# jimmc414/semantic_merge

Hardware: AMD Instinct MI355X
Metric: op-log compose+conflict throughput (ops/s), 100M-op logs, 1/2/4/8 GPUs (higher is better)
Workload: dtype u64; 1 GPU; c3: one merge of 100,000,000 ops (100,000,000 per GPU), 1,000,000 symbols, 64 ops/ms, seed 11; n_ops_per_gpu=100000000, n_ops_total=100000000, n_sym=1000000, composed_ops=99989720, conflicts=5140, plan=presorted, parallelism=single GPU

## Files before the change

semantic_merge_amd/csrc/smx_compose.hip:

```cpp
#include <algorithm>
#include <atomic>
#include <chrono>
#include <cstring>
#include <mutex>
#include <string>
#include <vector>

#include "smx_sort.h"
#include "smx_window.h"
#include "smx_small.h"
#include "smx_batch.h"
#include "smx_tables.h"


static thread_local std::string g_err;
static int set_err(int code, const std::string& msg) {
  g_err = msg;
  return code;
}
int smx_set_error(int code, const char* msg) { return set_err(code, msg ? msg : ""); }
#define HIP_TRY(x)                                                                 \
  do {                                                                             \
    hipError_t _e = (x);                                                           \
    if (_e != hipSuccess)                                                          \
// ... 1052 lines not shown
  const u64 nskip = M->n_skip;
  const u64 nmv = min(M->kcnt[KMOVE], E.n);
  const u64 nP = E.n - nmv;
  const u64 nR = min(M->kcnt[KREN], nP);
  const u64 nout = E.n - nskip, nRk = nR - nskip;
  auto gsrc = [&](i32 j) -> i32 {
    if (E.src_map) return E.src_map[j];
    return (u64)j < E.na_loc ? (i32)(E.src_a + j) : (i32)(E.src_b + ((i64)j - (i64)E.na_loc));
  };
  const FinPack FP = fin_pack_of(M->vbits, E.allow_pack != 0);
  const int lane = threadIdx.x & (WAVE - 1);
  const u64 w0 = (((u64)blockIdx.x * BLOCK + threadIdx.x) / WAVE) * EMIT_WT;
  if (w0 + EMIT_WT <= nmv || w0 >= nout || nP == 0) return;
  u64 kk = 0;
  {
    const u64 o0 = w0 > nmv ? w0 - nmv : 0;
    if (o0 < nRk) {
      u64 lo = 0, hi = nskip;
      while (lo < hi) {
        const u64 mid = (lo + hi) >> 1;
        if ((u64)E.skiplist[mid] - mid < o0) lo = mid + 1;
        else hi = mid;
      }
      kk = lo;
    }
  }
  u64 pp[EMIT4_STEPS][4];
  bool vec[EMIT4_STEPS];
#pragma unroll
  for (int j = 0; j < EMIT4_STEPS; ++j) {
    const u64 b = w0 + (u64)j * 4 * WAVE;
    const u64 o = b + 4 * (u64)lane;
    u64 add[4] = {0, 0, 0, 0};
    const u64 k0 = kk;
    if (b + 4 * WAVE > nmv && (b > nmv ? b - nmv : 0) < nRk) {
      const u64 ohi = b + 4 * WAVE - 1 - nmv;
      while (kk < nskip) {
        const u64 sj = (u64)(u32)__builtin_amdgcn_readfirstlane((int)E.skiplist[kk]) - kk;
        if (sj > ohi) break;
#pragma unroll
        for (int u = 0; u < 4; ++u) add[u] += (o + u >= nmv ? o + u - nmv : 0) >= sj;
        ++kk;
      }
    }
#pragma unroll
    for (int u = 0; u < 4; ++u) {
      const u64 ou = o + u;
      const u64 op = ou >= nmv ? ou - nmv : 0;
      const bool ok = ou >= nmv && ou < nout;
      pp[j][u] = !ok ? 0 : (op < nRk ? op + k0 + add[u] : op + nskip);
    }
    vec[j] = o >= nmv && o + 3 < nout && pp[j][3] == pp[j][0] + 3;
  }
  i32 src[EMIT4_STEPS][4];
  u32 sy[EMIT4_STEPS][4];
#pragma unroll
  for (int j = 0; j < EMIT4_STEPS; ++j) {
    if (vec[j]) {
      const ev4u s4 = __builtin_nontemporal_load(reinterpret_cast<const ev4u_a4*>(&E.tsrc[pp[j][0]]));
      const ev4u y4 = __builtin_nontemporal_load(reinterpret_cast<const ev4u_a4*>(&E.tsym[pp[j][0]]));
      src[j][0] = (i32)s4.x, src[j][1] = (i32)s4.y, src[j][2] = (i32)s4.z, src[j][3] = (i32)s4.w;
      sy[j][0] = y4.x, sy[j][1] = y4.y, sy[j][2] = y4.z, sy[j][3] = y4.w;
    } else {
#pragma unroll
      for (int u = 0; u < 4; ++u) {
        src[j][u] = NTLD(&E.tsrc[pp[j][u]]);
        sy[j][u] = NTLD(&E.tsym[pp[j][u]]);
      }
    }
#pragma unroll
    for (int u = 0; u < 4; ++u) sy[j][u] = min(sy[j][u], E.smax);
  }
#pragma unroll
  for (int j = 0; j < EMIT4_STEPS; ++j) {
    int4 F[4];
    if (FP.packed) {
      u64 x[4];
#pragma unroll
      for (int u = 0; u < 4; ++u) x[u] = fin_word(FP, E.fin, sy[j][u]);
#pragma unroll
      for (int u = 0; u < 4; ++u) F[u] = fin_decode(FP, x[u]);
    } else {
#pragma unroll
      for (int u = 0; u < 4; ++u) F[u] = E.fin[sy[j][u]];
    }
    const u64 o = w0 + (u64)j * 4 * WAVE + 4 * (u64)lane;
    i32 vo[4], va[4], vf[4], vc[4];
#pragma unroll
    for (int u = 0; u < 4; ++u) {
      const bool ren = o + u >= nmv && o + u - nmv < nRk;
      vo[u] = gsrc(src[j][u]);
      va[u] = F[u].x;
      vf[u] = F[u].y;
      vc[u] = ren ? -1 : F[u].z;
    }
    if (o >= nmv && o + 3 < nout) {
      NTST((ev4i{vo[0], vo[1], vo[2], vo[3]}), reinterpret_cast<ev4i*>(&E.out_order[o]));
      NTST((ev4i{va[0], va[1], va[2], va[3]}), reinterpret_cast<ev4i*>(&E.out_addr[o]));
      NTST((ev4i{vf[0], vf[1], vf[2], vf[3]}), reinterpret_cast<ev4i*>(&E.out_file[o]));
      NTST((ev4i{vc[0], vc[1], vc[2], vc[3]}), reinterpret_cast<ev4i*>(&E.out_ctx[o]));
    } else {
#pragma unroll
      for (int u = 0; u < 4; ++u) {
        if (o + u >= nmv && o + u < nout) {
          E.out_order[o + u] = vo[u];
          E.out_addr[o + u] = va[u];
          E.out_file[o + u] = vf[u];
          E.out_ctx[o + u] = vc[u];
        }
      }
    }
  }
}

__global__ void k_mv_init(const u32* __restrict__ msym, u64 nMv, u64* __restrict__ keys, u32* __restrict__ vals) {
  for (u64 j = (u64)blockIdx.x * BLOCK + threadIdx.x; j < nMv; j += (u64)gridDim.x * BLOCK) {
    keys[j] = msym[j] & SYM_MASK;
    vals[j] = (u32)j;
  }
}

__global__ void k_mv_fix(const u64* __restrict__ keys, const u32* __restrict__ vals, u64 nMv,
                         const u32* __restrict__ msym, const u64* __restrict__ mvpre, u64 n_sym,
                         i32* __restrict__ out_addr, i32* __restrict__ out_file) {
  for (u64 j = (u64)blockIdx.x * BLOCK + threadIdx.x; j < nMv; j += (u64)gridDim.x * BLOCK) {
    if (j != 0 && keys[j - 1] == keys[j]) continue;
    i32 ra = -1, rf = -1;
    if (mvpre && keys[j] < n_sym) {
      const u64 pa = mvpre[keys[j]], pf = mvpre[n_sym + keys[j]];
      if (pa) ra = (i32)(u32)pa - 1;
      if (pf) rf = (i32)(u32)pf - 1;
    }
    for (u64 i = j; i < nMv && keys[i] == keys[j]; ++i) {
      const u32 T = vals[i];
      const u32 f = msym[T];
      if (f & MS_HAS_A) ra = out_addr[T];
      else out_addr[T] = ra;
      if (f & MS_HAS_F) rf = out_file[T];
      else out_file[T] = rf;
    }
  }
}


struct Layout {
  size_t off[64];
  size_t total;
};

enum Buf {
  B_META, B_BND, B_WCNT, B_WOFF, B_STS, B_SHI, B_SLO, B_PERM, B_RKEY, B_RVAL, B_RK2, B_RV2,
  B_RHIST, B_PART, B_MSYM, B_TSRC, B_TSYM, B_RSTR, B_WREN, B_WBND, B_CSLOT, B_WCAND, B_WCANDB,
  B_WCOFF, B_CAND, B_Q, B_PM, B_NCONF, B_NREAL, B_COFF, B_SKIPBITS, B_SKIPLIST,
  B_TABA, B_TABF, B_TABR, B_FIN, B_REC, B_TBHIST, B_CCNT, B_TSUM, B_SMP, B_N
};

static i64 max_windows(i64 nn) { return SMX_CEIL_DIV(nn, (i64)WIN_TGT_MIN) + 2; }

static Layout layout(i64 na, i64 nb, i64 n_sym) {
  const i64 n = na + nb;
  const i64 nn = n > 0 ? n : 1;
  const i64 W = max_windows(nn);
  size_t sz[B_N];
  sz[B_META] = sizeof(ComposeMeta);
  sz[B_BND] = (size_t)(W + 1) * 2 * 8;
  sz[B_WCNT] = (size_t)NCNT * W * 4;
  sz[B_WOFF] = (size_t)NCNT * W * 4;
  sz[B_STS] = sz[B_SHI] = sz[B_SLO] = (size_t)nn * 8;
  sz[B_PERM] = (size_t)nn * 4;
  sz[B_RKEY] = (size_t)nn * 8;
  sz[B_RVAL] = (size_t)nn * 4;
  sz[B_RK2] = (size_t)nn * 8;
  sz[B_RV2] = (size_t)nn * 4;
  sz[B_RHIST] = radix_hist_bytes(nn);
  sz[B_PART] = (size_t)SCAN_NB * 8;
  sz[B_MSYM] = sz[B_TSRC] = sz[B_TSYM] = sz[B_RSTR] = (size_t)nn * 4;
  sz[B_WREN] = (size_t)W * 2 * 4;
  sz[B_WBND] = sz[B_WCAND] = sz[B_WCANDB] = sz[B_WCOFF] = (size_t)W * 4;
  sz[B_CSLOT] = sz[B_CAND] = sz[B_Q] = sz[B_PM] = sz[B_NCONF] = sz[B_NREAL] = sz[B_COFF] = (size_t)nn * 4;
  sz[B_SKIPBITS] = (size_t)(SMX_CEIL_DIV(nn, (i64)64) + 1) * 8;
  sz[B_SKIPLIST] = (size_t)nn * 4;
  const i64 ns = n_sym > 0 ? n_sym : 1;
  sz[B_TABA] = sz[B_TABF] = sz[B_TABR] = (size_t)ns * 4;
  sz[B_FIN] = (size_t)ns * 16;
  sz[B_REC] = (size_t)nn * 4;
  sz[B_TBHIST] = (size_t)(TB_MAXBK + 1) * SMX_CEIL_DIV(nn, (i64)TB_TILE) * 4;
  sz[B_CCNT] = (size_t)2 * SMX_N_KINDS * (SMX_CEIL_DIV(nn, (i64)256) + 2) * 4;
  sz[B_SMP] = (size_t)(SMX_CEIL_DIV(nn, (i64)CH) + 4) * 8;
  sz[B_TSUM] = (size_t)2 * SMX_N_KINDS * (SMX_CEIL_DIV(nn, (i64)CH * CS_TILE) + 2) * 4;
  Layout L{};
  size_t acc = 0;
  for (int i = 0; i < B_N; ++i) {
    L.off[i] = acc;
    acc += (sz[i] + 255) & ~(size_t)255;
  }
  L.total = acc;
  return L;
}


static int grid_for(i64 n, int per_block_items = BLOCK) {
  i64 g = SMX_CEIL_DIV(n > 0 ? n : 1, (i64)per_block_items);
  if (g > 4096) g = 4096;
  return (int)g;
}

extern "C" int smx_compose_workspace_bytes(int64_t n_a, int64_t n_b, int64_t n_sym, size_t* bytes) {
  if (!bytes || n_a < 0 || n_b < 0 || n_sym < 0) return set_err(SMX_E_ARG, "bad argument");
  *bytes = layout(n_a, n_b, n_sym).total;
  return SMX_OK;
}

struct Ctx {
  const smx_ops* ops;
  const smx_compose_out* out;
  hipStream_t st;
  Layout L{};
  char* base;
  i64 na, nb, n, n_sym;
  i64 src_a, src_b;
  StageTimer* tm;
  const i32* src_map = nullptr;
  u64* hrec = nullptr;
  u64 hseq = 0;
  template <typename T>
  T* ws(int b) const { return (T*)(base + L.off[b]); }
};

#if SMX_DIAG
static void* g_phase_dbg = nullptr;
static size_t g_phase_dbg_bytes = 0;
extern "C" int smx_debug_phase_buffer(void* p, size_t bytes) {
  g_phase_dbg = p;
  g_phase_dbg_bytes = bytes;
  return SMX_OK;
}
#else
static constexpr void* g_phase_dbg = nullptr;
static constexpr size_t g_phase_dbg_bytes = 0;
#endif

static WinArgs win_args(const Ctx& C) {
  WinArgs P{};
  P.kind = C.ops->kind;
  P.sym = C.ops->sym;
  P.v0 = C.ops->v0;
  P.v1 = C.ops->v1;
  P.na = C.na;
  P.nb = C.nb;
  P.bgap = C.ops->b_gap;
  P.n_sym = C.n_sym;
  P.src_a = C.src_a;
  P.src_b = C.src_b;
  P.src_map = C.src_map;
  P.bnd = C.ws<i64>(B_BND);
  P.woff = C.ws<u32>(B_WOFF);
  P.meta = C.ws<ComposeMeta>(B_META);
  P.out_order = C.out->order;
  P.out_addr = C.out->addr;
  P.out_file = C.out->file;
  P.out_ctx = C.out->ctx;
  P.msym = C.ws<u32>(B_MSYM);
  P.tsrc = C.ws<i32>(B_TSRC);
  P.tsym = C.ws<u32>(B_TSYM);
  P.Rstr = C.ws<i32>(B_RSTR);
  P.wren = C.ws<u32>(B_WREN);
  P.wbnd = C.ws<u32>(B_WBND);
  P.cslot = C.ws<u32>(B_CSLOT);
  P.wcand = C.ws<u32>(B_WCAND);
  return P;
}

static WalkArgs walk_args(const Ctx& C, const smx_shard* sh) {
  WalkArgs Wk{};
  Wk.tsrc = C.ws<i32>(B_TSRC);
  Wk.tsym = C.ws<u32>(B_TSYM);
  Wk.v0 = C.ops->v0;
  Wk.wren = C.ws<u32>(B_WREN);
  Wk.wbnd = C.ws<u32>(B_WBND);
  Wk.meta = C.ws<ComposeMeta>(B_META);
  Wk.na_cap = (u64)C.na;
  Wk.nb_cap = (u64)C.nb;
  Wk.bgap = C.ops->b_gap;
  Wk.src_a = C.src_a;
  Wk.src_b = C.src_b;
  Wk.src_map = C.src_map;
  Wk.halo_dev = sh ? sh->halo_dev : nullptr;
  for (int b = 0; b < 2; ++b) {
    Wk.halo_sym[b] = sh ? sh->halo_sym[b] : nullptr;
    Wk.halo_cls[b] = sh ? sh->halo_cls[b] : nullptr;
    Wk.halo_src[b] = sh ? sh->halo_src[b] : nullptr;
    Wk.halo_n[b] = sh && sh->halo_sym[b] ? (u64)sh->halo_n[b] : 0;
    Wk.halo_more[b] = sh ? sh->halo_more[b] : 0;
  }
  Wk.stage = C.ws<u32>(B_RK2);
  Wk.sok = C.ws<u32>(B_RV2);
  Wk.stage_cap = RS_CONF ? (u64)(C.n > 0 ? C.n : 1) * 2 / (RS_CONF ? RS_W : 1) : 0;
  return Wk;
}

#ifndef SMX_WALK_LB
#define SMX_WALK_LB 0
#endif
static int launch_walk(const Ctx& C, const smx_shard* sh) {
  hipStream_t st = C.st;
  ComposeMeta* meta = C.ws<ComposeMeta>(B_META);
  const i64 n = C.n;
  u64* skipbits = C.ws<u64>(B_SKIPBITS);
  u32* skiplist = C.ws<u32>(B_SKIPLIST);
  u32* part = C.ws<u32>(B_PART);
  const u64 nskipw = (u64)SMX_CEIL_DIV(n, (i64)64) + 1;
  const WalkArgs Wk = walk_args(C, sh);
  u32* cslot = C.ws<u32>(B_CSLOT);
  u32* wcand = C.ws<u32>(B_WCAND);
  u32* wtot = C.ws<u32>(B_WCANDB);
  u32* wcoff = C.ws<u32>(B_WCOFF);
  u32* cand = C.ws<u32>(B_CAND);
  u32* q = C.ws<u32>(B_Q);
  u32* pm = C.ws<u32>(B_PM);
  u32* nconf = C.ws<u32>(B_NCONF);
  u32* nreal = C.ws<u32>(B_NREAL);
  u32* coff = C.ws<u32>(B_COFF);
  u32* nconf32 = (u32*)&meta->n_conf_loc;
  u32* ncand32 = (u32*)&meta->n_cand;
  const u64* ncand_dev = &meta->n_cand;
  const i64 Wmax = max_windows(n);
#ifndef WALK_GSMALL
#define WALK_GSMALL 256
#endif
  const int gsmall = WALK_GSMALL;
  const bool lb_cc = SMX_WALK_LB && !sh && Wmax <= WALK_CC_FUSED_MAXW;
  const bool lb_cl = SMX_WALK_LB && !sh && n <= WALK_FUSED_MAXN;
  if (lb_cc)
    hipLaunchKernelGGL(k_boundary_cc, dim3(grid_for(Wmax)), dim3(BLOCK), 0, st, Wk, meta, cslot, wcand, wtot,
                       skipbits, nskipw, wcoff, (u64)Wmax, ncand32, cand);
  else
    hipLaunchKernelGGL(k_boundary, dim3(grid_for(Wmax)), dim3(BLOCK), 0, st, Wk, meta, cslot, wcand, wtot, skipbits,
// ... 45 lines not shown
  A.ncap = (u64)C.n;
  A.width = 1u;
  A.nbk = 1u;
  A.smax = (u32)(C.n_sym - 1);
  return A;
}

static bool tb_geometry(const Ctx& C, u64* width_o, u64* nbk_o) {
  u64 width = SMX_CEIL_DIV((u64)C.n_sym, (u64)TB_NBK_TGT);
  if (width < 1) width = 1;
  if (width > TB_WIDTH) width = TB_WIDTH;
  *width_o = width;
  *nbk_o = SMX_CEIL_DIV((u64)C.n_sym, width);
  return *nbk_o <= TB_MAXBK;
}

static int launch_tb_prescatter(const Ctx& C) {
  u64 width, nbk;
  if (!tb_geometry(C, &width, &nbk)) return SMX_OK;
  TbArgs A = tb_args(C);
  A.width = (u32)width;
  A.nbk = (u32)nbk;
  A.keep_skip = 1u;
  hipLaunchKernelGGL(k_tb_scatter, dim3((int)SMX_CEIL_DIV((u64)C.n, (u64)TB_TILE)), dim3(TB_NT), 0, C.st, A,
                     C.ws<u32>(B_TBHIST), C.ws<u32>(B_REC));
  HIP_TRY(hipGetLastError());
  return SMX_OK;
}

static int launch_tables(const Ctx& C, void* part_tab, u32 tag, int tagbits, bool* bucketed,
                         bool prescattered = false) {
  hipStream_t st = C.st;
  const i64 n = C.n;
  int4* fin = C.ws<int4>(B_FIN);
  *bucketed = false;
  const i64 n_sym = C.n_sym;
  TbArgs A = tb_args(C);
  u64 width, nbk;
  if (tb_geometry(C, &width, &nbk)) {
    *bucketed = true;
    A.width = (u32)width;
    A.nbk = (u32)nbk;
    const int nblk = (int)SMX_CEIL_DIV((u64)n, (u64)TB_TILE);
    u32* lst = C.ws<u32>(B_TBHIST);
    u32* rec = C.ws<u32>(B_REC);
    if (prescattered) {
      A.keep_skip = 1u;
      hipLaunchKernelGGL(k_tb_unskip, dim3(1024), dim3(BLOCK), 0, st, A, lst, rec, C.ws<u32>(B_SKIPLIST));
    } else {
      hipLaunchKernelGGL(k_tb_scatter, dim3(nblk), dim3(TB_NT), 0, st, A, lst, rec);
    }
    hipLaunchKernelGGL(k_tb_reduce, dim3(nbk), dim3(TBR_NT), 0, st, A, lst, rec, n_sym, fin,
                       PartTab{part_tab, tag, tagbits, C.ws<ComposeMeta>(B_META)});
  } else {
    u32* tabA = C.ws<u32>(B_TABA);
    u32* tabF = C.ws<u32>(B_TABF);
    u32* tabR = C.ws<u32>(B_TABR);
    int rc;
    if ((rc = zero_async(tabA, (size_t)n_sym * 4, st)) || (rc = zero_async(tabF, (size_t)n_sym * 4, st)) ||
        (rc = zero_async(tabR, (size_t)n_sym * 4, st)))
      return rc;
    hipLaunchKernelGGL(k_tab_atomic, dim3(grid_for(n)), dim3(BLOCK), 0, st, A, tabA, tabF, tabR);
    hipLaunchKernelGGL(k_finalize, dim3(grid_for(n_sym)), dim3(BLOCK), 0, st, A, tabA, tabF, tabR, n_sym, fin,
                       PartTab{part_tab, tag, tagbits, C.ws<ComposeMeta>(B_META)});
  }
  HIP_TRY(hipGetLastError());
  return SMX_OK;
}

static int launch_emit(const Ctx& C, bool packable, const smx_shard* sh) {
  hipStream_t st = C.st;
  ComposeMeta* meta = C.ws<ComposeMeta>(B_META);
  const i64 n = C.n;
  EmitArgs E{C.ws<i32>(B_TSRC), C.ws<u32>(B_TSYM), C.ws<u64>(B_SKIPBITS), C.ws<u32>(B_SKIPLIST),
             C.ws<int4>(B_FIN), meta, (u64)n, (u32)(C.n_sym - 1), packable ? 1 : 0, (u64)C.na, C.src_a,
             C.src_b, C.src_map, C.out->order, C.out->addr, C.out->file, C.out->ctx, C.out->counts, sh ? 0 : 1,
             sh ? nullptr : C.hrec, C.hseq};
  const i64 ewaves = SMX_CEIL_DIV(n, (i64)EMIT_WT);
  const bool al16 = ((uintptr_t)C.out->order | (uintptr_t)C.out->addr | (uintptr_t)C.out->file |
                     (uintptr_t)C.out->ctx) % 16 == 0;
  if (EMIT_VEC && al16)
    hipLaunchKernelGGL(k_emit4, dim3(SMX_CEIL_DIV(ewaves, (i64)NWAVES)), dim3(BLOCK), 0, st, E);
  else
    hipLaunchKernelGGL(k_emit, dim3(SMX_CEIL_DIV(ewaves, (i64)NWAVES)), dim3(BLOCK), 0, st, E);
  HIP_TRY(hipGetLastError());
  return SMX_OK;
}

#if SMX_DIAG
static int knob(const char* name, int dflt) {
  const char* v = getenv(name);
  return v && *v ? atoi(v) : dflt;
}
#else
static constexpr int knob(const char*, int dflt) { return dflt; }
#endif

struct SideStream {
  std::mutex mu;
  int dev = -1;
  hipStream_t caller = nullptr;
  hipStream_t s = nullptr;
  hipEvent_t fork = nullptr, join = nullptr;
};
#define SIDE_MAX 256
static std::mutex g_side_mu;
static SideStream* g_side[SIDE_MAX];
static int g_nside = 0;

static int side_stream(hipStream_t caller, SideStream** out) {
  *out = nullptr;
  int dev = 0;
  HIP_TRY(hipGetDevice(&dev));
  std::lock_guard<std::mutex> g(g_side_mu);
  for (int i = 0; i < g_nside; ++i)
    if (g_side[i]->dev == dev && g_side[i]->caller == caller) {
      *out = g_side[i];
      return SMX_OK;
    }
  if (g_nside == SIDE_MAX) return SMX_OK;
  SideStream* S = new SideStream;
  S->dev = dev;
  S->caller = caller;
  int ncu = 0;
  HIP_TRY(hipDeviceGetAttribute(&ncu, hipDeviceAttributeMultiprocessorCount, dev));
  const int k = knob("SMX_SIDE_CUS", 0);
  if (k > 0 && k < ncu) {
    std::vector<uint32_t> mask((size_t)(ncu + 31) / 32, 0u);
    for (int i = 0; i < k; ++i) mask[(size_t)i / 32] |= 1u << (i % 32);
    HIP_TRY(hipExtStreamCreateWithCUMask(&S->s, (uint32_t)mask.size(), mask.data()));
  } else {
    HIP_TRY(hipStreamCreateWithFlags(&S->s, hipStreamNonBlocking));
  }
#ifndef SMX_SIDE_SYSFENCE
#define SMX_SIDE_SYSFENCE 0
#endif
  const unsigned evf = hipEventDisableTiming | (SMX_SIDE_SYSFENCE ? 0u : hipEventDisableSystemFence);
  HIP_TRY(hipEventCreateWithFlags(&S->fork, evf));
  HIP_TRY(hipEventCreateWithFlags(&S->join, evf));
  g_side[g_nside++] = S;
  *out = S;
  return SMX_OK;
}

#ifndef SMX_TB_OVERLAP
#define SMX_TB_OVERLAP 1
#endif
#ifndef SMX_TB_UNSKIP_MAXN
#define SMX_TB_UNSKIP_MAXN (1 << 22)
#endif
#ifndef SMX_TB_OVERLAP_MIN
#define SMX_TB_OVERLAP_MIN (1 << 18)
#endif
static bool n_side_needed(const smx_ops* ops) {
  u64 width = SMX_CEIL_DIV((u64)ops->n_sym, (u64)TB_NBK_TGT);
  if (width < 1) width = 1;
  if (width > TB_WIDTH) width = TB_WIDTH;
  return SMX_TB_OVERLAP && SMX_CEIL_DIV((u64)ops->n_sym, width) <= TB_MAXBK &&
         ops->n_a + ops->n_b >= SMX_TB_OVERLAP_MIN;
}

static int launch_tail(const Ctx& C) {
  const i64 n_sym = C.n_sym;
  u64 width = SMX_CEIL_DIV((u64)n_sym, (u64)TB_NBK_TGT);
  if (width < 1) width = 1;
  if (width > TB_WIDTH) width = TB_WIDTH;
  const u64 nbk = SMX_CEIL_DIV((u64)n_sym, width);
  SideStream* S = nullptr;
  if (SMX_TB_OVERLAP && nbk <= TB_MAXBK && C.n >= SMX_TB_OVERLAP_MIN && !knob("SMX_TB_SERIAL", 0)) {
    int rc = side_stream(C.st, &S);
    if (rc) return rc;
  }
  if (!S) {
    C.tm->begin(ST_WALK);
    int rc = launch_walk(C, nullptr);
    if (rc) return rc;
    C.tm->end(ST_WALK);
    C.tm->begin(ST_TABLES);
    bool bucketed = false;
    if ((rc = launch_tables(C, nullptr, 0, 0, &bucketed))) return rc;
    C.tm->end(ST_TABLES);
    C.tm->begin(ST_EMIT);
    if ((rc = launch_emit(C, bucketed, nullptr))) return rc;
    C.tm->end(ST_EMIT);
    return SMX_OK;
  }
  std::lock_guard<std::mutex> own(S->mu);
  int rc;
  hipStream_t st = C.st;
  TbArgs A = tb_args(C);
  A.width = (u32)width;
  A.nbk = (u32)nbk;
  A.keep_skip = C.n <= SMX_TB_UNSKIP_MAXN ? 2u : 1u;
  u32* lst = C.ws<u32>(B_TBHIST);
  u32* rec = C.ws<u32>(B_REC);
  const int nblk = (int)SMX_CEIL_DIV((u64)C.n, (u64)TB_TILE);
  HIP_TRY(hipEventRecord(S->fork, st));
  HIP_TRY(hipStreamWaitEvent(S->s, S->fork, 0));
  hipLaunchKernelGGL(k_tb_scatter, dim3(nblk), dim3(TB_NT), 0, S->s, A, lst, rec);
  HIP_TRY(hipGetLastError());
  HIP_TRY(hipEventRecord(S->join, S->s));
  C.tm->begin(ST_WALK);
  if ((rc = launch_walk(C, nullptr))) {
    (void)hipStreamWaitEvent(st, S->join, 0);
    return rc;
  }
  C.tm->end(ST_WALK);
  HIP_TRY(hipStreamWaitEvent(st, S->join, 0));
  C.tm->begin(ST_TABLES);
  if (A.keep_skip == 1u)
    hipLaunchKernelGGL(k_tb_unskip, dim3(1024), dim3(BLOCK), 0, st, A, lst, rec, C.ws<u32>(B_SKIPLIST));
  hipLaunchKernelGGL(k_tb_reduce, dim3(nbk), dim3(TBR_NT), 0, st, A, lst, rec, n_sym, C.ws<int4>(B_FIN),
                     PartTab{nullptr, 0u, 0, nullptr});
  HIP_TRY(hipGetLastError());
  C.tm->end(ST_TABLES);
  C.tm->begin(ST_EMIT);
  if ((rc = launch_emit(C, true, nullptr))) return rc;
  C.tm->end(ST_EMIT);
  return SMX_OK;
}


struct EarlyFail {
  u32* flag_host = nullptr;
  u32* flag_dev = nullptr;
  hipEvent_t ev = nullptr;
};
enum WinLevel { WL_SMALL, WL_NORMAL, WL_WIDE };
static i64 level_cap(int lv) { return lv == WL_SMALL ? WF_SMALL_CAP : lv == WL_WIDE ? WF_WIDE_CAP : WF_CAP; }
static int first_level(const Ctx& C) {
  if (knob("SMX_FIRST_WIDE", 0)) return WL_WIDE;
  return C.n <= WF_SMALL_MAXN ? WL_SMALL : WL_NORMAL;
}
static i64 first_tgt(const Ctx& C) {
  if (first_level(C) == WL_WIDE) return knob("SMX_WIN_TGT", WF_WIDE_CAP);
  return first_level(C) == WL_SMALL ? knob("SMX_WIN_TGT", WF_SMALL_TGT) : knob("SMX_WIN_TGT", WIN_TGT);
}

static int launch_presorted_windows(const Ctx& C, i64 W, i64 CM, int level) {
  const bool wide = level == WL_WIDE;
  hipStream_t st = C.st;
  WinArgs P = win_args(C);
  P.cpre = C.ws<u32>(B_CCNT);
  P.CM = CM;
  P.kts = C.ops->ts;
  P.khi = C.ops->oid_hi;
  P.klo = C.ops->oid_lo;
  P.perm = nullptr;
  P.W = W;
  P.ablate = knob("SMX_ABLATE", 0);
  const int stage = wide ? ST_WINDOW_WIDE : ST_WINDOW;
  C.tm->begin(stage);
#if SMX_DIAG
  if (g_phase_dbg && !P.src_map && (size_t)W * WF_NSTAMP * 8 <= g_phase_dbg_bytes) {
    P.dbg = (u64*)g_phase_dbg;
    if (wide)
      hipLaunchKernelGGL((k_window_f<WF_WIDE_CAP, WF_WIDE_NT, true, false>), dim3(W), dim3(WF_WIDE_NT), 0, st, P);
    else
      hipLaunchKernelGGL((k_window_f<WF_CAP, WF_NT, true, false>), dim3(W), dim3(WF_NT), 0, st, P);
  } else
#endif
  if (wide) {
    if (P.src_map) hipLaunchKernelGGL((k_window_f<WF_WIDE_CAP, WF_WIDE_NT, false, true, WF_RUNS_WIDE>), dim3(W), dim3(WF_WIDE_NT), 0, st, P);
    else hipLaunchKernelGGL((k_window_f<WF_WIDE_CAP, WF_WIDE_NT, false, false, WF_RUNS_WIDE>), dim3(W), dim3(WF_WIDE_NT), 0, st, P);
  } else if (level == WL_SMALL) {
    if (P.src_map) hipLaunchKernelGGL((k_window_f<WF_SMALL_CAP, WF_SMALL_NT, false, true>), dim3(W), dim3(WF_SMALL_NT), 0, st, P);
    else hipLaunchKernelGGL((k_window_f<WF_SMALL_CAP, WF_SMALL_NT, false, false>), dim3(W), dim3(WF_SMALL_NT), 0, st, P);
  } else if (P.src_map) {
    hipLaunchKernelGGL((k_window_f<WF_CAP, WF_NT, false, true, WF_RUNS>), dim3(W), dim3(WF_NT), 0, st, P);
  } else {
    hipLaunchKernelGGL((k_window_f<WF_CAP, WF_NT, false, false, WF_RUNS>), dim3(W), dim3(WF_NT), 0, st, P);
  }
  HIP_TRY(hipGetLastError());
  C.tm->end(stage);
  return SMX_OK;
}



struct Deferred {
  bool on = false;
  i64 W = 0, W_w = 0, CM = 0;
};
static int run_presorted(const Ctx& C, i64 tgt, const EarlyFail* early = nullptr, int level = WL_NORMAL,
                         Deferred* defer = nullptr) {
  hipStream_t st = C.st;
  ComposeMeta* meta = C.ws<ComposeMeta>(B_META);
  i64* bnd = C.ws<i64>(B_BND);
  C.tm->begin(ST_PLAN);
  static_assert(sizeof(ComposeMeta) % 4 == 0, "meta is zeroed by words");
  if (tgt < WIN_TGT_MIN) tgt = WIN_TGT_MIN;
  const i64 cap = level_cap(level);
  if (tgt > cap) tgt = cap;
  tgt -= tgt % CH;
  const i64 W = SMX_CEIL_DIV(C.n, tgt);
  const i64 CM = SMX_CEIL_DIV(C.na > C.nb ? C.na : C.nb, (i64)CH) + 1;
  const bool cs_small = CM <= CS_SMALL_CM;
  {
    const int rc = zero_async(meta, sizeof(ComposeMeta), st);
    if (rc) return rc;
  }
  const i64 nchunk = SMX_CEIL_DIV(C.na, (i64)CH) + SMX_CEIL_DIV(C.nb, (i64)CH);
  u32* ccnt = C.ws<u32>(B_CCNT);
  u64* sA = C.ws<u64>(B_SMP);
  u64* sB = sA + SMX_CEIL_DIV(C.na, (i64)CH) + 1;
  const bool lmode = early && defer && level == WL_NORMAL && !KH_PERSIST;
  LongW lw{};
  if (lmode) {
    lw.tgt_w = level_cap(WL_WIDE) - level_cap(WL_WIDE) % CH;
    lw.W_w = SMX_CEIL_DIV(C.n, lw.tgt_w);
    lw.D_w = level_cap(WL_WIDE) / CH;
  }
  if (KH_PERSIST) {
    static int ncu_of[64] = {};
    int dev = 0;
    HIP_TRY(hipGetDevice(&dev));
    int ncu = dev < 64 ? ncu_of[dev] : 0;
    if (ncu == 0) {
      HIP_TRY(hipDeviceGetAttribute(&ncu, hipDeviceAttributeMultiprocessorCount, dev));
      if (dev < 64) ncu_of[dev] = ncu;
    }
    const i64 ngrp = SMX_CEIL_DIV(nchunk, (i64)CH_PER_BLOCK);
    const i64 grid = ngrp < (i64)ncu * KH_BLOCKS_PER_CU ? ngrp : (i64)ncu * KH_BLOCKS_PER_CU;
    hipLaunchKernelGGL(k_khist2, dim3(grid > 0 ? grid : 1), dim3(KH_NT), 0, st, C.ops->kind, C.ops->ts, C.na, C.nb,
                       C.ops->b_gap, CM, ccnt, sA, sB, meta, early ? early->flag_dev : nullptr);
  } else {
    hipLaunchKernelGGL(k_khist, dim3(SMX_CEIL_DIV(nchunk, (i64)CH_PER_BLOCK * KH_R)), dim3(KH_NT), 0, st,
                       C.ops->kind, C.ops->ts, C.na, C.nb, C.ops->b_gap, CM, ccnt, sA, sB, meta,
                       early ? early->flag_dev : nullptr, lmode ? cap / CH : (i64)0);
  }
  if (lmode) HIP_TRY(hipEventRecord(early->ev, st));
  const i64 nfp = SMX_CEIL_DIV(W + 1, (i64)BLOCK);
  const bool fused = SMX_FPART_CS && cs_small && !early;
  if (fused)
    hipLaunchKernelGGL(k_fpart_cscan, dim3(nfp + 2 * SMX_N_KINDS), dim3(BLOCK), 0, st, C.ops->ts,
                       C.ops->ts + C.na + C.ops->b_gap, sA, sB, C.na, C.nb, W, tgt, cap / CH, bnd, meta,
                       (u32*)nullptr, ccnt, CM, nfp);
  else
    hipLaunchKernelGGL(k_fpart, dim3(nfp), dim3(BLOCK), 0, st, C.ops->ts, C.ops->ts + C.na + C.ops->b_gap, sA, sB,
                       C.na, C.nb, W, tgt, cap / CH, bnd, meta, (early && !lmode) ? early->flag_dev : nullptr, lw);
  if (early && !lmode) HIP_TRY(hipEventRecord(early->ev, st));
  const u64 nwin_long = lmode ? (u64)lw.W_w : 0ull;
  if (fused) {
  } else if (cs_small) {
    hipLaunchKernelGGL(k_cscan_small, dim3(2 * SMX_N_KINDS), dim3(BLOCK), 0, st, ccnt, C.na, C.nb, CM, meta, (u64)W,
                       nwin_long);
  } else {
    const i64 NT = SMX_CEIL_DIV(CM, (i64)CS_TILE);
    u32* tsum = C.ws<u32>(B_TSUM);
    hipLaunchKernelGGL(k_cscan_up, dim3(NT, 2 * SMX_N_KINDS), dim3(BLOCK), 0, st, ccnt, C.na, C.nb, CM, NT, tsum,
                       meta);
    hipLaunchKernelGGL(k_cscan_mid, dim3(2 * SMX_N_KINDS), dim3(BLOCK), 0, st, tsum, C.na, C.nb, CM, NT, ccnt,
                       meta, (u64)W, nwin_long);
    hipLaunchKernelGGL(k_cscan_down, dim3(NT, 2 * SMX_N_KINDS), dim3(BLOCK), 0, st, ccnt, C.na, C.nb, CM, NT,
                       tsum, meta);
  }
  HIP_TRY(hipGetLastError());
  C.tm->end(ST_PLAN);
  if (lmode) {
    *defer = Deferred{true, W, lw.W_w, CM};
    return SMX_OK;
  }
  return launch_presorted_windows(C, W, CM, level);
}

__global__ void k_plan_rearm(ComposeMeta* meta, u64 nwin) {
// ... 1206 lines not shown
```

semantic_merge_amd/csrc/smx_tables.h:

```cpp
#pragma once

#include "smx_scan.h"

#define TB_WIDTH 4096
#define TB_MAXBK 1024
#ifndef TB_NT
#define TB_NT 1024
#endif
#define TB_NW (TB_NT / WAVE)
#ifndef TB_ITEMS
#define TB_ITEMS 16
#endif
#ifndef TB_NBK_TGT
#define TB_NBK_TGT 256
#endif
#define TB_TILE (TB_NT * TB_ITEMS)
#define REC_IB (TB_TILE <= (1 << 14) ? 14 : 15)
static_assert(TB_TILE <= (1 << 15), "tile-relative record index is at most 15 bits");
#define REC_IMASK ((1u << REC_IB) - 1u)
#define REC_HAS_A (1u << (REC_IB + 12))
#define REC_HAS_F (1u << (REC_IB + 13))

struct TbArgs {
  const u32* msym;
// ... 53 lines not shown
    }
  } else if (base >= A.nMv && end <= nrec) {
    u32 s[TB_ITEMS];
    const u64 m0 = base - A.nMv;
#pragma unroll
    for (int it = 0; it < TB_ITEMS; ++it) s[it] = A.tsym[m0 + (u64)it * TB_NT + threadIdx.x];
#pragma unroll
    for (int it = 0; it < TB_ITEMS; ++it) {
      ok[it] = A.keep_skip || !tb_skipped(A, m0 + (u64)it * TB_NT + threadIdx.x);
      fl[it] = 0;
      sym[it] = min(s[it], A.smax);
    }
  } else {
#pragma unroll
    for (int it = 0; it < TB_ITEMS; ++it) {
      const u64 r = base + (u64)it * TB_NT + threadIdx.x;
      ok[it] = r < nrec && tb_record(A, r, &sym[it], &fl[it]);
    }
  }
}

__global__ void __launch_bounds__(TB_NT) k_tb_scatter(TbArgs A0, u32* __restrict__ lst, u32* __restrict__ rec) {
  __shared__ u32 stage[TB_TILE];
  __shared__ u32 lstart[TB_MAXBK];
  __shared__ u32 wsum[TB_NW + 1];
  const TbArgs A = tb_load(A0);
  const u64 nrec = A.nMv + A.nR;
  const u64 base = (u64)blockIdx.x * TB_TILE;
  if (base >= nrec) return;
  const u32 nbk = A.nbk;
  for (u32 i = threadIdx.x; i < nbk; i += TB_NT) lstart[i] = 0;
  __syncthreads();
  u32 q[TB_ITEMS];
  u32 bk[TB_ITEMS];
  {
    u32 s[TB_ITEMS], fl[TB_ITEMS];
    bool ok[TB_ITEMS];
    tb_items(A, base, s, fl, ok);
#pragma unroll
    for (int it = 0; it < TB_ITEMS; ++it) {
      const u32 loc = (u32)(it * TB_NT) + threadIdx.x;
      bk[it] = 0xffffffffu;
      if (ok[it]) {
        const u32 b = s[it] / A.width;
        bk[it] = b;
        q[it] = loc | ((s[it] - b * A.width) << REC_IB) | fl[it];
        atomicAdd(&lstart[b], 1u);
      }
    }
  }
  __syncthreads();
  u32* lt = lst + (u64)blockIdx.x * (nbk + 1);
  {
    u32 v[TB_MAXBK / TB_NT];
    u32 acc = 0;
#pragma unroll
    for (int j = 0; j < TB_MAXBK / TB_NT; ++j) {
      const u32 b = threadIdx.x * (TB_MAXBK / TB_NT) + j;
      v[j] = b < nbk ? lstart[b] : 0u;
      acc += v[j];
    }
    u32 tot;
    u32 run = block_excl_scan<OpSum, u32, TB_NW>(acc, wsum, &tot);
#pragma unroll
    for (int j = 0; j < TB_MAXBK / TB_NT; ++j) {
      const u32 b = threadIdx.x * (TB_MAXBK / TB_NT) + j;
      if (b < nbk) {
        lstart[b] = run;
        lt[b] = run;
      }
      run += v[j];
    }
    if (threadIdx.x == 0) {
      wsum[TB_NW] = tot;
      lt[nbk] = tot;
    }
  }
  __syncthreads();
  const u32 total = wsum[TB_NW];
#pragma unroll
  for (int it = 0; it < TB_ITEMS; ++it) {
    if (bk[it] == 0xffffffffu) continue;
    const u32 pos = atomicAdd(&lstart[bk[it]], 1u);
    stage[pos] = q[it];
  }
  __syncthreads();
  for (u32 i = threadIdx.x; i < total; i += TB_NT) rec[base + i] = stage[i];
}

#define REC_DEAD 0xffffffffu
__global__ void k_tb_unskip(TbArgs A0, const u32* __restrict__ lst, u32* __restrict__ rec,
                            const u32* __restrict__ skiplist) {
  const TbArgs A = tb_load(A0);
  const u64 nskip = min(A.meta->n_skip, A.nR);
  const u32 nb1 = A.nbk + 1;
  const u32 lane = threadIdx.x & (WAVE - 1);
  const u64 nwv = (u64)gridDim.x * (blockDim.x / WAVE);
  for (u64 i = (u64)blockIdx.x * (blockDim.x / WAVE) + threadIdx.x / WAVE; i < nskip; i += nwv) {
    const u64 m = skiplist[i];
    if (m >= A.nR) continue;
    const u64 r = A.nMv + m;
    const u64 tile = r / TB_TILE;
    const u32 loc = (u32)(r - tile * TB_TILE);
    const u32 sym = min(A.tsym[m], A.smax);
    const u32 b = sym / A.width;
    const u32* lt = lst + tile * nb1;
    const u64 rb = tile * TB_TILE;
    const u32 e = lt[b + 1];
    for (u32 j = lt[b] + lane; j < e; j += WAVE) {
      const u32 q = rec[rb + j];
      if (q != REC_DEAD && (q & REC_IMASK) == loc) rec[rb + j] = REC_DEAD;
    }
  }
}

#define TBR_NT 1024
#ifndef SMX_XCD_TB
#define SMX_XCD_TB 1
#endif
#ifndef TBR_TK
#define TBR_TK 16
#endif
#ifndef TBR_U
#define TBR_U 2
#endif
#ifndef TBR_PREFETCH
#define TBR_PREFETCH 1
#endif

struct PartTab {
  void* p;
  u32 tag;
  int tagbits;
  ComposeMeta* meta;
  __device__ __forceinline__ void put(i64 n_sym, i64 s, int va, int vf, int vc) const {
    if (tagbits == 0) {
      u64* part = (u64*)p;
      const u64 tg = (u64)tag << 32;
      part[s] = va >= 0 ? tg | (u32)(va + 1) : 0ull;
      part[n_sym + s] = vf >= 0 ? tg | (u32)(vf + 1) : 0ull;
      part[2 * n_sym + s] = vc >= 0 ? tg | (u32)(vc + 1) : 0ull;
      return;
    }
    u32* part = (u32*)p;
    const u32 vb = 31u - (u32)tagbits, tg = tag << vb, lim = 1u << vb;
    const u32 a1 = (u32)(va + 1), f1 = (u32)(vf + 1), c1 = (u32)(vc + 1);
    if ((a1 | f1 | c1) >= lim) meta->tab_over = 1;
    part[s] = va >= 0 ? tg | (a1 & (lim - 1)) : 0u;
    part[n_sym + s] = vf >= 0 ? tg | (f1 & (lim - 1)) : 0u;
    part[2 * n_sym + s] = vc >= 0 ? tg | (c1 & (lim - 1)) : 0u;
  }
};

__global__ void __launch_bounds__(TBR_NT) k_tb_reduce(TbArgs A0, const u32* __restrict__ lst,
                                                      const u32* __restrict__ rec, i64 n_sym,
                                                      int4* __restrict__ fin, PartTab part) {
  const FinPack FP = fin_pack_of(A0.meta->vbits, true);
  __shared__ u32 tA[TB_WIDTH], tF[TB_WIDTH], tC[TB_WIDTH];
  const TbArgs A = tb_load(A0);
  const u32 b = SMX_XCD_TB ? (u32)xcd_item(blockIdx.x, gridDim.x) : blockIdx.x;
  for (u32 i = threadIdx.x; i < A.width; i += TBR_NT) tA[i] = tF[i] = tC[i] = 0;
  __syncthreads();
  auto put = [&](u32 q, u64 rb) {
    const u32 r1 = (u32)(rb + (q & REC_IMASK)) + 1u;
    const u32 ls = (q >> REC_IB) & 0xfffu;
    if ((u64)(r1 - 1) < A.nMv) {
      if (q & REC_HAS_A) atomicMax(&tA[ls], r1);
      if (q & REC_HAS_F) atomicMax(&tF[ls], r1);
    } else if (A.keep_skip != 2u || !tb_skipped(A, (u64)(r1 - 1) - A.nMv)) {
      atomicMax(&tC[ls], r1);
    }
  };
  const u64 nrec = A.nMv + A.nR;
  const int nt = nrec ? (int)SMX_CEIL_DIV(nrec, (u64)TB_TILE) : 0;
  const int lane = threadIdx.x & (WAVE - 1), wv = threadIdx.x / WAVE;
  const u32 nb1 = A.nbk + 1;
  constexpr int NW = TBR_NT / WAVE;
  auto bounds = [&](int t0, u32* lo, u32* hi) {
    *lo = *hi = 0;
    if (lane < TBR_TK && t0 + lane < nt) {
      const u32* lt = lst + (u64)(t0 + lane) * nb1;
      *lo = lt[b];
      *hi = lt[b + 1];
    }
  };
  u32 lo_n = 0, hi_n = 0;
  if (TBR_PREFETCH) bounds(wv * TBR_TK, &lo_n, &hi_n);
  for (int t0 = wv * TBR_TK; t0 < nt; t0 += NW * TBR_TK) {
    u32 lo = lo_n, hi = hi_n;
    if (!TBR_PREFETCH) bounds(t0, &lo, &hi);
    u32 q[TBR_TK][TBR_U];
#pragma unroll
    for (int k = 0; k < TBR_TK; ++k) {
      const u32 lk = __builtin_amdgcn_readlane(lo, k), hk = __builtin_amdgcn_readlane(hi, k);
      const u64 rb = (u64)(t0 + k) * TB_TILE;
#pragma unroll
      for (int u = 0; u < TBR_U; ++u) {
        const u32 i = lk + (u32)lane + (u32)(u * WAVE);
        q[k][u] = i < hk ? __builtin_nontemporal_load(&rec[rb + i]) : ~0u;
      }
    }
    if (TBR_PREFETCH) bounds(t0 + NW * TBR_TK, &lo_n, &hi_n);
#pragma unroll
    for (int k = 0; k < TBR_TK; ++k)
#pragma unroll
      for (int u = 0; u < TBR_U; ++u)
        if (q[k][u] != ~0u) put(q[k][u], (u64)(t0 + k) * TB_TILE);
#pragma unroll
    for (int k = 0; k < TBR_TK; ++k) {
      const u32 lk = __builtin_amdgcn_readlane(lo, k), hk = __builtin_amdgcn_readlane(hi, k);
      const u64 rb = (u64)(t0 + k) * TB_TILE;
      for (u32 i = lk + TBR_U * WAVE + (u32)lane; i < hk; i += WAVE) {
        const u32 x = rec[rb + i];
        if (x != REC_DEAD) put(x, rb);
      }
    }
  }
  __syncthreads();
  const u32 s0 = b * A.width;
  for (u32 i = threadIdx.x; i < A.width && (i64)(s0 + i) < n_sym; i += TBR_NT) {
    const u32 a = tA[i], f = tF[i], c = tC[i];
    const int va = a ? A.mv_addr[a - 1] : -1, vf = f ? A.mv_file[f - 1] : -1;
    const int vc = c ? A.Rstr[(u64)(c - 1) - A.nMv] : -1;
    if (part.p) part.put(n_sym, s0 + i, va, vf, vc);
    else fin_put(FP, fin, s0 + i, va, vf, vc);
  }
}

__global__ void k_tab_atomic(TbArgs A0, u32* __restrict__ tabA, u32* __restrict__ tabF, u32* __restrict__ tabR) {
  const TbArgs A = tb_load(A0);
  const u64 nrec = A.nMv + A.nR;
  for (u64 r = (u64)blockIdx.x * BLOCK + threadIdx.x; r < nrec; r += (u64)gridDim.x * BLOCK) {
    u32 s, fl;
    if (!tb_record(A, r, &s, &fl)) continue;
    const u32 r1 = (u32)r + 1u;
    if (r < A.nMv) {
      if (fl & REC_HAS_A) atomicMax(&tabA[s], r1);
      if (fl & REC_HAS_F) atomicMax(&tabF[s], r1);
    } else {
      atomicMax(&tabR[s], r1);
    }
  }
}

__global__ void k_finalize(TbArgs A0, const u32* __restrict__ tabA, const u32* __restrict__ tabF,
                           const u32* __restrict__ tabR, i64 n_sym, int4* __restrict__ fin, PartTab part) {
  const TbArgs A = tb_load(A0);
  for (i64 s = (i64)blockIdx.x * BLOCK + threadIdx.x; s < n_sym; s += (i64)gridDim.x * BLOCK) {
    const u32 a = tabA[s], f = tabF[s], c = tabR[s];
    const int va = a ? A.mv_addr[a - 1] : -1, vf = f ? A.mv_file[f - 1] : -1;
    const int vc = c ? A.Rstr[(u64)(c - 1) - A.nMv] : -1;
    if (part.p) part.put(n_sym, s, va, vf, vc);
    else fin[s] = make_int4(va, vf, vc, 0);
  }
}
```

Measured before the change: 42.48 billion ops/s.

## Split table reduce into move pass on side stream and rename pass

```diff
diff --git a/semantic_merge_amd/csrc/smx_compose.hip b/semantic_merge_amd/csrc/smx_compose.hip
--- a/semantic_merge_amd/csrc/smx_compose.hip
+++ b/semantic_merge_amd/csrc/smx_compose.hip
@@ -1228,7 +1228,7 @@
   B_META, B_BND, B_WCNT, B_WOFF, B_STS, B_SHI, B_SLO, B_PERM, B_RKEY, B_RVAL, B_RK2, B_RV2,
   B_RHIST, B_PART, B_MSYM, B_TSRC, B_TSYM, B_RSTR, B_WREN, B_WBND, B_CSLOT, B_WCAND, B_WCANDB,
   B_WCOFF, B_CAND, B_Q, B_PM, B_NCONF, B_NREAL, B_COFF, B_SKIPBITS, B_SKIPLIST,
-  B_TABA, B_TABF, B_TABR, B_FIN, B_REC, B_TBHIST, B_CCNT, B_TSUM, B_SMP, B_N
+  B_TABA, B_TABF, B_TABR, B_FIN, B_MVV, B_REC, B_TBHIST, B_CCNT, B_TSUM, B_SMP, B_N
 };
 
 static i64 max_windows(i64 nn) { return SMX_CEIL_DIV(nn, (i64)WIN_TGT_MIN) + 2; }
@@ -1259,6 +1259,7 @@
   const i64 ns = n_sym > 0 ? n_sym : 1;
   sz[B_TABA] = sz[B_TABF] = sz[B_TABR] = (size_t)ns * 4;
   sz[B_FIN] = (size_t)ns * 16;
+  sz[B_MVV] = (size_t)ns * 8;
   sz[B_REC] = (size_t)nn * 4;
   sz[B_TBHIST] = (size_t)(TB_MAXBK + 1) * SMX_CEIL_DIV(nn, (i64)TB_TILE) * 4;
   sz[B_CCNT] = (size_t)2 * SMX_N_KINDS * (SMX_CEIL_DIV(nn, (i64)256) + 2) * 4;
@@ -1610,6 +1611,9 @@
 #ifndef SMX_TB_OVERLAP_MIN
 #define SMX_TB_OVERLAP_MIN (1 << 18)
 #endif
+#ifndef SMX_TB_SPLIT
+#define SMX_TB_SPLIT 1
+#endif
 static bool n_side_needed(const smx_ops* ops) {
   u64 width = SMX_CEIL_DIV((u64)ops->n_sym, (u64)TB_NBK_TGT);
   if (width < 1) width = 1;
@@ -1656,6 +1660,8 @@
   HIP_TRY(hipEventRecord(S->fork, st));
   HIP_TRY(hipStreamWaitEvent(S->s, S->fork, 0));
   hipLaunchKernelGGL(k_tb_scatter, dim3(nblk), dim3(TB_NT), 0, S->s, A, lst, rec);
+  int2* mvv = C.ws<int2>(B_MVV);
+  if (SMX_TB_SPLIT) hipLaunchKernelGGL(k_tb_reduce_mv, dim3(nbk), dim3(TBR_NT), 0, S->s, A, lst, rec, n_sym, mvv);
   HIP_TRY(hipGetLastError());
   HIP_TRY(hipEventRecord(S->join, S->s));
   C.tm->begin(ST_WALK);
@@ -1668,8 +1674,11 @@
   C.tm->begin(ST_TABLES);
   if (A.keep_skip == 1u)
     hipLaunchKernelGGL(k_tb_unskip, dim3(1024), dim3(BLOCK), 0, st, A, lst, rec, C.ws<u32>(B_SKIPLIST));
-  hipLaunchKernelGGL(k_tb_reduce, dim3(nbk), dim3(TBR_NT), 0, st, A, lst, rec, n_sym, C.ws<int4>(B_FIN),
-                     PartTab{nullptr, 0u, 0, nullptr});
+  if (SMX_TB_SPLIT)
+    hipLaunchKernelGGL(k_tb_reduce_rn, dim3(nbk), dim3(TBR_NT), 0, st, A, lst, rec, n_sym, C.ws<int4>(B_FIN), mvv);
+  else
+    hipLaunchKernelGGL(k_tb_reduce, dim3(nbk), dim3(TBR_NT), 0, st, A, lst, rec, n_sym, C.ws<int4>(B_FIN),
+                       PartTab{nullptr, 0u, 0, nullptr});
   HIP_TRY(hipGetLastError());
   C.tm->end(ST_TABLES);
   C.tm->begin(ST_EMIT);
diff --git a/semantic_merge_amd/csrc/smx_tables.h b/semantic_merge_amd/csrc/smx_tables.h
--- a/semantic_merge_amd/csrc/smx_tables.h
+++ b/semantic_merge_amd/csrc/smx_tables.h
@@ -229,27 +229,39 @@
   }
 };
 
-__global__ void __launch_bounds__(TBR_NT) k_tb_reduce(TbArgs A0, const u32* __restrict__ lst,
-                                                      const u32* __restrict__ rec, i64 n_sym,
-                                                      int4* __restrict__ fin, PartTab part) {
+enum { TBR_BOTH = 0, TBR_MOVES = 1, TBR_RENAMES = 2 };
+
+template <int PASS>
+__device__ __forceinline__ void tb_reduce_body(TbArgs A0, const u32* __restrict__ lst, const u32* __restrict__ rec,
+                                               i64 n_sym, int4* __restrict__ fin, PartTab part, int2* mvv) {
+  constexpr bool MV = PASS != TBR_RENAMES, RN = PASS != TBR_MOVES;
   const FinPack FP = fin_pack_of(A0.meta->vbits, true);
-  __shared__ u32 tA[TB_WIDTH], tF[TB_WIDTH], tC[TB_WIDTH];
+  __shared__ u32 tab[(MV ? 2 : 0) + (RN ? 1 : 0)][TB_WIDTH];
+  u32* const tA = tab[0];
+  u32* const tF = tab[MV ? 1 : 0];
+  u32* const tC = tab[MV && RN ? 2 : 0];
   const TbArgs A = tb_load(A0);
   const u32 b = SMX_XCD_TB ? (u32)xcd_item(blockIdx.x, gridDim.x) : blockIdx.x;
-  for (u32 i = threadIdx.x; i < A.width; i += TBR_NT) tA[i] = tF[i] = tC[i] = 0;
+  for (u32 i = threadIdx.x; i < A.width; i += TBR_NT) {
+    if (MV) tA[i] = tF[i] = 0;
+    if (RN) tC[i] = 0;
+  }
   __syncthreads();
   auto put = [&](u32 q, u64 rb) {
     const u32 r1 = (u32)(rb + (q & REC_IMASK)) + 1u;
     const u32 ls = (q >> REC_IB) & 0xfffu;
     if ((u64)(r1 - 1) < A.nMv) {
-      if (q & REC_HAS_A) atomicMax(&tA[ls], r1);
-      if (q & REC_HAS_F) atomicMax(&tF[ls], r1);
-    } else if (A.keep_skip != 2u || !tb_skipped(A, (u64)(r1 - 1) - A.nMv)) {
+      if (MV) {
+        if (q & REC_HAS_A) atomicMax(&tA[ls], r1);
+        if (q & REC_HAS_F) atomicMax(&tF[ls], r1);
+      }
+    } else if (RN && (A.keep_skip != 2u || !tb_skipped(A, (u64)(r1 - 1) - A.nMv))) {
       atomicMax(&tC[ls], r1);
     }
   };
-  const u64 nrec = A.nMv + A.nR;
-  const int nt = nrec ? (int)SMX_CEIL_DIV(nrec, (u64)TB_TILE) : 0;
+  const u64 rend = PASS == TBR_MOVES ? A.nMv : A.nMv + A.nR;
+  const int tlo = PASS == TBR_RENAMES ? (int)(A.nMv / (u64)TB_TILE) : 0;
+  const int nt = rend ? (int)SMX_CEIL_DIV(rend, (u64)TB_TILE) : 0;
   const int lane = threadIdx.x & (WAVE - 1), wv = threadIdx.x / WAVE;
   const u32 nb1 = A.nbk + 1;
   constexpr int NW = TBR_NT / WAVE;
@@ -262,8 +274,8 @@
     }
   };
   u32 lo_n = 0, hi_n = 0;
-  if (TBR_PREFETCH) bounds(wv * TBR_TK, &lo_n, &hi_n);
-  for (int t0 = wv * TBR_TK; t0 < nt; t0 += NW * TBR_TK) {
+  if (TBR_PREFETCH) bounds(tlo + wv * TBR_TK, &lo_n, &hi_n);
+  for (int t0 = tlo + wv * TBR_TK; t0 < nt; t0 += NW * TBR_TK) {
     u32 lo = lo_n, hi = hi_n;
     if (!TBR_PREFETCH) bounds(t0, &lo, &hi);
     u32 q[TBR_TK][TBR_U];
@@ -296,12 +308,41 @@
   __syncthreads();
   const u32 s0 = b * A.width;
   for (u32 i = threadIdx.x; i < A.width && (i64)(s0 + i) < n_sym; i += TBR_NT) {
-    const u32 a = tA[i], f = tF[i], c = tC[i];
-    const int va = a ? A.mv_addr[a - 1] : -1, vf = f ? A.mv_file[f - 1] : -1;
+    int va, vf;
+    if (MV) {
+      const u32 a = tA[i], f = tF[i];
+      va = a ? A.mv_addr[a - 1] : -1;
+      vf = f ? A.mv_file[f - 1] : -1;
+    } else {
+      const int2 v = mvv[s0 + i];
+      va = v.x;
+      vf = v.y;
+    }
+    if (PASS == TBR_MOVES) {
+      mvv[s0 + i] = make_int2(va, vf);
+      continue;
+    }
+    const u32 c = tC[i];
     const int vc = c ? A.Rstr[(u64)(c - 1) - A.nMv] : -1;
     if (part.p) part.put(n_sym, s0 + i, va, vf, vc);
     else fin_put(FP, fin, s0 + i, va, vf, vc);
   }
+}
+
+__global__ void __launch_bounds__(TBR_NT) k_tb_reduce(TbArgs A0, const u32* __restrict__ lst,
+                                                      const u32* __restrict__ rec, i64 n_sym,
+                                                      int4* __restrict__ fin, PartTab part) {
+  tb_reduce_body<TBR_BOTH>(A0, lst, rec, n_sym, fin, part, nullptr);
+}
+__global__ void __launch_bounds__(TBR_NT) k_tb_reduce_mv(TbArgs A0, const u32* __restrict__ lst,
+                                                         const u32* __restrict__ rec, i64 n_sym,
+                                                         int2* __restrict__ mvv) {
+  tb_reduce_body<TBR_MOVES>(A0, lst, rec, n_sym, nullptr, PartTab{nullptr, 0u, 0, nullptr}, mvv);
+}
+__global__ void __launch_bounds__(TBR_NT) k_tb_reduce_rn(TbArgs A0, const u32* __restrict__ lst,
+                                                         const u32* __restrict__ rec, i64 n_sym,
+                                                         int4* __restrict__ fin, const int2* __restrict__ mvv) {
+  tb_reduce_body<TBR_RENAMES>(A0, lst, rec, n_sym, fin, PartTab{nullptr, 0u, 0, nullptr}, const_cast<int2*>(mvv));
 }
 
 __global__ void k_tab_atomic(TbArgs A0, u32* __restrict__ tabA, u32* __restrict__ tabF, u32* __restrict__ tabR) {
```

Measured after the change: 42.86 billion ops/s, median of 6. Within noise of the previous version (+0.9%).
